# locuslab/icnn

Measured on AMD Instinct MI355X. Metric: inner-solves/sec (batch x iters), n=159 K=10, higher is better.
Workload: dtype f32 PICNN / f64 dual solve

## Files before the change

### icnn_amd/_lib.py

```python
import ctypes as C
import os

import torch

HERE = os.path.dirname(os.path.abspath(__file__))
LIB_PATH = os.path.join(HERE, "csrc", "libicnn_be.so")
if os.environ.get("ICNN_BE_LIB"):
    LIB_PATH = os.path.abspath(os.environ["ICNN_BE_LIB"])

ABI_VERSION = 12
MAX_LAYERS = 8
MAX_SLOTS = 31
MAX_ITERS = 64
MAX_ROUNDS = 128
VARIANT = {"dual": 0, "rl": 1, "pdipm": 2}
CUT_F32, CUT_F64 = 0, 1
ST_SINGULAR, ST_NONFINITE, ST_OVERFLOW, ST_UNFINISHED = 1, 2, 4, 8
ST_ERROR_MASK = ST_SINGULAR | ST_NONFINITE | ST_UNFINISHED | ST_OVERFLOW
FLAG_NO_CYCLE_SHORTCUT = 1
FLAG_TIME_SLICE = 2
FLAG_LOCKSTEP = 4
FLAG_TWO_KERNELS = 8
FLAG_PERSISTENT = 16
FLAG_F64_ENERGY = 32
# ... 8 lines not shown
DUAL_KERNELS = ["small", "body", "wide"]
ERRORS = {-1: "ICNN_BE_EINVAL (bad argument)", -2: "ICNN_BE_ELIMIT (size beyond a compiled-in limit)",
          -3: "ICNN_BE_ELAUNCH (HIP launch failed)"}

EXPORTS = [
    "icnn_be_abi_version", "icnn_be_last_hip_error", "icnn_be_struct_size", "icnn_be_dual_lds_bytes", "icnn_be_bundle_capacity", "icnn_be_scratch_bytes",
    "icnn_be_state_init",
    "icnn_be_dual_step", "icnn_be_fc_pack_floats", "icnn_be_fc_pack", "icnn_be_fc_fg",
    "icnn_be_solve_fc", "icnn_be_solve_fc_reset", "icnn_be_conv_pack_floats", "icnn_be_conv_work_floats", "icnn_be_conv_pack", "icnn_be_conv_fg", "icnn_be_solve_conv",
    "icnn_be_implicit_feed", "icnn_be_export_active", "icnn_be_adam_workspace_bytes", "icnn_be_adam_fc", "icnn_be_adam_fc_obs",
    "icnn_be_adam_fc_each", "icnn_be_debug_adam_each_plan",
    "icnn_be_fc_context_work_floats", "icnn_be_fc_context", "icnn_be_fc_context_stage", "icnn_be_fc_context_norm", "icnn_be_fc_clamp",
    "icnn_be_conv_context_work_floats", "icnn_be_conv_context", "icnn_be_conv_clamp",
    "icnn_be_debug_profile", "icnn_be_debug_profile_fc", "icnn_be_debug_profile_conv", "icnn_be_debug_profile_phases",
    "icnn_be_debug_fast_math", "icnn_be_debug_trace", "icnn_be_debug_solve_plan", "icnn_be_debug_adam_plan", "icnn_be_debug_dual_plan",
    "icnn_be_debug_shape_instance",
    "icnn_be_fc_grad_floats", "icnn_be_fc_surrogate_grad_work_floats", "icnn_be_fc_surrogate_grad",
    "icnn_be_conv_grad_floats", "icnn_be_conv_surrogate_grad_work_floats", "icnn_be_conv_surrogate_grad",
    "icnn_be_fc_context_bn_work_floats", "icnn_be_fc_context_bn", "icnn_be_conv_context_bn_work_floats", "icnn_be_conv_context_bn",
    "icnn_be_fc_surrogate_grad_bn", "icnn_be_conv_surrogate_grad_bn", "icnn_be_param_update",
    "icnn_be_gd_workspace_bytes", "icnn_be_fc_gd", "icnn_be_conv_gd",
    "icnn_be_rl_td", "icnn_be_rl_critic_update", "icnn_be_rl_bundle_solve",
    "icnn_be_ficnn_pack_floats", "icnn_be_ficnn_pack", "icnn_be_ficnn_context_work_floats", "icnn_be_ficnn_context",
    "icnn_be_ficnn_fg", "icnn_be_ficnn_gd", "icnn_be_solve_ficnn", "icnn_be_ficnn_grad_floats",
    "icnn_be_ficnn_surrogate_grad_work_floats", "icnn_be_ficnn_surrogate_grad",
    "icnn_be_feed_plan_work_bytes", "icnn_be_feed_plan", "icnn_be_feed_pad", "icnn_be_fc_surrogate_grad_dev",
    "icnn_be_conv_surrogate_grad_dev", "icnn_be_fc_context_bn_dev", "icnn_be_conv_context_bn_dev",
    "icnn_be_fc_surrogate_grad_dev_work_floats", "icnn_be_conv_surrogate_grad_dev_work_floats",
    "icnn_be_gd_feed_work_bytes", "icnn_be_gd_feed", "icnn_be_gd_feed_px_work_bytes", "icnn_be_gd_feed_px",
    "icnn_be_step_gate", "icnn_be_param_update_gated", "icnn_be_gated_copy",
    "icnn_be_replay_enqueue", "icnn_be_replay_sample",
# ... 283 lines not shown
    lib.icnn_be_implicit_feed.argtypes = [C.POINTER(State), C.c_void_p, C.c_int] + [C.c_void_p] * 6
    lib.icnn_be_implicit_feed.restype = C.c_int
    lib.icnn_be_export_active.argtypes = [C.POINTER(State)] + [C.c_void_p] * 6
    lib.icnn_be_export_active.restype = C.c_int
    lib.icnn_be_debug_fast_math.argtypes = [C.c_int, C.c_void_p, C.c_void_p, C.c_int, C.c_void_p]
    lib.icnn_be_debug_fast_math.restype = C.c_int
    lib.icnn_be_debug_solve_plan.argtypes = [C.POINTER(FcModel), C.POINTER(State), C.c_int, C.POINTER(C.c_int * 3)]
    lib.icnn_be_debug_solve_plan.restype = C.c_int
    lib.icnn_be_debug_profile_phases.restype = C.c_int
    lib.icnn_be_debug_adam_plan.argtypes = [C.POINTER(FcModel), C.POINTER(FcCtx), C.c_int, C.POINTER(C.c_int * 4)]
    lib.icnn_be_debug_adam_plan.restype = C.c_int
    lib.icnn_be_debug_dual_plan.argtypes = [C.POINTER(State), C.c_int, C.POINTER(C.c_int * 8)]
    lib.icnn_be_debug_dual_plan.restype = C.c_int
    lib.icnn_be_debug_shape_instance.argtypes = [C.POINTER(FcModel), C.POINTER(State)]
    lib.icnn_be_debug_shape_instance.restype = C.c_int
    lib.icnn_be_adam_workspace_bytes.argtypes = [C.c_int, C.c_int]
    lib.icnn_be_adam_workspace_bytes.restype = C.c_size_t
    lib.icnn_be_adam_fc.argtypes = [C.POINTER(FcModel), C.c_void_p, C.c_int, C.c_int] + [C.c_void_p] * 5
    lib.icnn_be_adam_fc.restype = C.c_int
    lib.icnn_be_adam_fc_each.argtypes = [C.POINTER(FcModel), C.c_void_p, C.c_int, C.c_int] + [C.c_void_p] * 5
    lib.icnn_be_adam_fc_each.restype = C.c_int
    lib.icnn_be_debug_adam_each_plan.argtypes = [C.POINTER(FcModel), C.c_int, C.POINTER(C.c_int * 2)]
    lib.icnn_be_debug_adam_each_plan.restype = C.c_int
    lib.icnn_be_adam_fc_obs.argtypes = [C.POINTER(FcModel), C.POINTER(FcCtx), C.c_void_p, C.c_int, C.c_int] + [C.c_void_p] * 5
    lib.icnn_be_adam_fc_obs.restype = C.c_int
    lib.icnn_be_fc_context_work_floats.argtypes = [C.POINTER(FcCtx), C.c_int]
    lib.icnn_be_fc_context_work_floats.restype = C.c_size_t
    lib.icnn_be_fc_context.argtypes = [C.POINTER(FcCtx), C.c_void_p, C.c_int, C.c_void_p, C.c_int, C.c_void_p, C.c_void_p]
    lib.icnn_be_fc_context.restype = C.c_int
    lib.icnn_be_fc_context_stage.argtypes = [C.POINTER(FcCtx), C.c_int, C.c_void_p, C.c_int, C.c_void_p, C.c_int, C.c_void_p,
# ... 260 lines not shown
def solve_plan(model, state, cus=0):
    out = (C.c_int * 3)()
    rc = load().icnn_be_debug_solve_plan(C.byref(model), C.byref(state), cus, C.byref(out))
    if rc < 0:
        check(rc, "icnn_be_debug_solve_plan")
    return (PATHS[rc],) + tuple(out)


def shape_instance(model, state):
    rc = load().icnn_be_debug_shape_instance(C.byref(model), C.byref(state))
    if rc < 0:
        check(rc, "icnn_be_debug_shape_instance")
    return SHAPE_INSTANCES[rc]


def adam_plan(model, batch, ctx=None):
    out = (C.c_int * 4)()
    rc = load().icnn_be_debug_adam_plan(C.byref(model), C.byref(ctx) if ctx is not None else None, int(batch), C.byref(out))
    if rc < 0:
        check(rc, "icnn_be_debug_adam_plan")
    return (ADAM_KERNELS[rc], out[0], out[1], bool(out[2]), bool(out[3]))


def adam_each_plan(model, batch):
    out = (C.c_int * 2)()
    rc = load().icnn_be_debug_adam_each_plan(C.byref(model), int(batch), C.byref(out))
    if rc < 0:
        check(rc, "icnn_be_debug_adam_each_plan")
    return (ADAM_KERNELS[rc], out[0], out[1])

# ... 9 lines not shown
```

### icnn_amd/csrc/be_api.hip

```cpp
#include <hip/hip_runtime.h>
#include <cmath>
#include <cstdlib>

#include <map>
#include <mutex>
#include <utility>

#include "be_api_check.h"
#include "be_kernels.h"
#include "icnn_be.h"

namespace {
thread_local hipError_t g_last = hipSuccess;

int fail(hipError_t e) {
    g_last = e;
    return e == hipErrorInvalidValue ? ICNN_BE_EINVAL : ICNN_BE_ELAUNCH;
}

int done(hipError_t e) { return e == hipSuccess ? 0 : fail(e); }
}

int icnn_be::api_done(hipError_t e) { return done(e); }

// ... 322 lines not shown
                                                    static_cast<hipStream_t>(stream), false,
                                                    icnn_be::SolveReset{1, nullptr, y0_fill}, &value);
    return e == hipSuccess ? p.rounds : fail(e);
}

int icnn_be_debug_solve_plan(const icnn_be_fc_model *model, const icnn_be_state *st, int cus, int out[3]) {
    if (!out) return ICNN_BE_EINVAL;
    if (int rc = check_fc_solve(model, st)) return rc;
    if (st->batch == 0) return ICNN_BE_EINVAL;
    const SolvePlan p = plan_fc_solve(*model, *st, cus > 0 ? cus : icnn_be::device_cus(), env_tile_budget());
    if (p.path < 0) return p.path;
    out[0] = p.per_wg; out[1] = p.budget; out[2] = p.rounds;
    return p.path;
}

int icnn_be_debug_shape_instance(const icnn_be_fc_model *model, const icnn_be_state *st) {
    if (model && st && st->cut_dtype == ICNN_BE_CUT_F64 && check_shape(st) == 0 && st->n == model->n && st->batch > 0 &&
        icnn_be::fc_check_model(*model) == 0)
        return ICNN_BE_SHAPE_GENERIC;
    if (int rc = check_fc_solve(model, st)) return rc;
    if (st->batch == 0) return ICNN_BE_EINVAL;
    const SolvePlan p = plan_fc_solve(*model, *st, icnn_be::device_cus(), env_tile_budget());
    if (p.path < 0) return p.path;
    if (p.path != ICNN_BE_PATH_TILE) return ICNN_BE_SHAPE_GENERIC;
    return icnn_be::fused_shape_instance(*model, *st, p.per_wg, p.budget);
}

size_t icnn_be_fc_context_work_floats(const icnn_be_fc_ctx *c, int batch) {
    if (!c || batch < 0 || icnn_be::ctx_check(*c) != 0) return 0;
    return icnn_be::ctx_work_floats(*c, batch);
// ... 505 lines not shown
```

### icnn_amd/csrc/be_fused.hip

```cpp
#include "be_dual_dev.h"
#include "be_dual_small_dev.h"
#include "be_picnn_fc_dev.h"
#include "be_picnn_fc_rows_dev.h"

namespace icnn_be {

namespace {

static_assert(NWAVE == TM, "one wave per sample in the dual phase");

struct FusedArgs {
    DualArgs da;
    FcArgs fa;
    int rounds, crow_off, samples_off, sample_bytes;
    int grouped;
    int group_cap, need_off;
    long long *trace;
    SolveReset reset;
};
typedef const __attribute__((address_space(4))) FusedArgs KArgs;

__device__ __forceinline__ void reset_sample(const icnn_be_state &st, const SolveReset &rs, int u, int lane) {
    const int n = st.n;
    double *yr = st.y + (size_t)u * n;
// ... 350 lines not shown
        !make_dual_args(args.da, st, nullptr, nullptr, 0, budget, st.slots, nullptr))
        return ICNN_BE_SHAPE_GENERIC;
    return pick_shape_instance(args, lay);
}

hipError_t launch_fused_fc_solve(const icnn_be_fc_model &m, const float *ctx, const icnn_be_state &st, float *f_work,
                                 float *g_work, long long *dual_prof, hipStream_t stream, int tile_rows, int budget,
                                 const SolveReset &reset) {
    if (budget > 0 && reset.on) return hipErrorInvalidValue;
    FusedTileLayout lay;
    if (!fused_tile_layout(m, st, tile_rows, budget, lay)) return hipErrorInvalidValue;
    FusedArgs args{};
    int fg_bytes = 0;
    if (fill_args(m, args.fa, fg_bytes) != 0) return hipErrorInvalidValue;
    args.fa.ctx = ctx; args.fa.y = st.y; args.fa.f = f_work; args.fa.g = g_work; args.fa.finished = st.skip_fg;
    args.fa.batch = st.batch; args.fa.prof = nullptr; args.fa.tile_rows = tile_rows;
    if (!make_dual_args(args.da, st, f_work, g_work, 0, budget, st.slots, dual_prof)) return hipErrorInvalidValue;
    args.rounds = st.iters > 0 ? st.iters : st.slots;
    args.crow_off = lay.crow_off; args.samples_off = 0; args.sample_bytes = lay.sample_bytes;
    args.grouped = lay.grouped; args.group_cap = lay.group_cap; args.need_off = lay.need_off;
    args.trace = dual_trace_buffer();
    args.reset = reset;
    const bool rl = st.variant == ICNN_BE_VARIANT_RL, big = st.slots > 15;
    auto kern = big ? (rl ? fused_fc_solve_kernel<true, 32> : fused_fc_solve_kernel<false, 32>)
                    : (rl ? fused_fc_solve_kernel<true, 16> : fused_fc_solve_kernel<false, 16>);
    if (st.variant == ICNN_BE_VARIANT_PDIPM) kern = big ? fused_fc_solve_kernel<false, 32, true> : fused_fc_solve_kernel<false, 16, true>;
    if (budget > 0) kern = big ? fused_fc_solve_kernel<false, 32, false, true> : fused_fc_solve_kernel<false, 16, false, true>;
    switch (pick_shape_instance(args, lay)) {
    case ICNN_BE_SHAPE_BIBTEX_KT16: kern = fused_fc_solve_kernel<false, 16, false, false, BibtexShape, 0>; break;
    case ICNN_BE_SHAPE_BIBTEX_KT32_GROUPED: kern = fused_fc_solve_kernel<false, 32, false, false, BibtexShape, 1>; break;
    default: break;
// ... 6 lines not shown
```

### icnn_amd/csrc/be_kernels.h

```cpp
#pragma once
#include <hip/hip_runtime.h>

#include "be_common.h"
#include "icnn_be.h"

namespace icnn_be {

struct DualArgs {
    icnn_be_state st;
    const void *f;
    const void *g;
    int round;
    int budget;
    int n_pad;
    int ldA;
    int rows;
    long long *prof;
    PairwisePlan plan;
};
constexpr int DUAL_PROF_PHASES = 16;
void set_dual_profile_buffer(long long *buf);
void set_fc_profile_buffer(long long *buf);
void set_conv_profile_buffer(long long *buf);

// ... 71 lines not shown
bool dual_step_small_fits(const icnn_be_state &st, int budget);
hipError_t launch_dual_step_small(const icnn_be_state &st, int round, const void *f, const void *g, hipStream_t stream);
struct DualStepPlan {
    int cut, kt, waves, variant, staged, kernel, lds, rows;
};
bool plan_dual_step(const icnn_be_state &st, int round, DualStepPlan &p);
void plan_dual_step_small(const icnn_be_state &st, DualStepPlan &p);

hipError_t launch_fast_math(int which, const double *x, double *out, int count, hipStream_t stream);
hipError_t launch_export_active(const icnn_be_state &st, const int *row_offset, void *G_rows, double *ys_rows, double *h_rows,
                                double *lam_rows, hipStream_t stream);
hipError_t launch_implicit_feed(const icnn_be_state &st, const double *y_true, int loss, const int *row_offset,
                                double *fd_y, double *fd_v, double *fd_c, int *fd_sample, hipStream_t stream);

int fc_check_model(const icnn_be_fc_model &m);
size_t fc_pack_floats(const icnn_be_fc_model &m);
int fc_pack(const icnn_be_fc_model &m, const float *const *w_yu, const float *const *w_zu, float *out);
hipError_t launch_fc_fg(const icnn_be_fc_model &m, const float *ctx, const double *y, int batch,
                        float *f, float *g, const int *finished, hipStream_t stream);

int ctx_check(const icnn_be_fc_ctx &c);
int conv_ctx_check(const icnn_be_conv_ctx &c);
size_t ctx_work_floats(const icnn_be_fc_ctx &c, int batch);
int ctx_stage_cols(const icnn_be_fc_ctx &c, int i);
int ctx_stage_ld(const icnn_be_fc_ctx &c, int i);
float *fc_ctx_u(const icnn_be_fc_ctx &c, int batch, float *work, int i, int *ld);
void fc_bn_widths(const icnn_be_fc_ctx &c, int *n);
hipError_t launch_fc_context(const icnn_be_fc_ctx &c, const float *x, int batch, float *ctx, int ctx_width, float *work,
                             hipStream_t stream, const icnn_be_bn_moving *mv = nullptr, int mode = ICNN_BE_BN_BATCH,
                             int updates = 0, const int *updates_dev = nullptr);
// ... 159 lines not shown
```

### icnn_amd/csrc/be_picnn_fc.hip

```cpp
#include "be_picnn_fc_dev.h"
#include "be_picnn_fc_rows_dev.h"

namespace icnn_be {

namespace {

__global__ __launch_bounds__(NTHREADS) void fc_fg_kernel(FcArgs a) {
    extern __shared__ __attribute__((aligned(16))) float lds[];
    fc_fg_tile(a, blockIdx.x, lds);
}

struct FgRowsArgs {
    FcArgs fa;
    RowsLayout lay;
    int per_wg;
};
__global__ __launch_bounds__(RTHREADS) void fc_fg_rows_kernel(FgRowsArgs a) {
#pragma clang fp contract(off)
    extern __shared__ __attribute__((aligned(16))) float lds[];
    const FcArgs &fa = a.fa;
    const int tid = threadIdx.x, wave = tid >> 6, lane = tid & 63;
    const int n = fa.n, RF = a.lay.row_floats;
    const int s_base = blockIdx.x * a.per_wg;
    const int batch = fa.batch - s_base < a.per_wg ? fa.batch - s_base : a.per_wg;
// ... 80 lines not shown
            if (e != hipSuccess) return e;
        } else {
            hipError_t e = launch_clamp(w + o.zu_f[i], (size_t)pad16(m.width[i - 1]), mode, stream);
            if (e != hipSuccess) return e;
        }
    }
    return hipSuccess;
}

int fc_check_model(const icnn_be_fc_model &m) {
    FcArgs a{};
    int lds = 0;
    return fill_args(m, a, lds);
}

}
```

### icnn_amd/csrc/be_picnn_fc_dev.h

```cpp
#pragma once
#include <hip/hip_runtime.h>

#include "be_common.h"
#include "be_kernels.h"
#include "icnn_be.h"

namespace icnn_be {

namespace {

constexpr int TM = 16;
constexpr int NWAVE = 16;
constexpr int NTHREADS = NWAVE * 64;

__host__ __device__ constexpr int pad16(int v) { return (v + 15) & ~15; }

struct FcArgs {
    int n, L;
    int width[ICNN_BE_MAX_LAYERS];
    float alpha;
    int action_box;
    int ctx_width;
    int yu_off[ICNN_BE_MAX_LAYERS], zu_off[ICNN_BE_MAX_LAYERS], gate_off[ICNN_BE_MAX_LAYERS];
    long long w_yu_f[ICNN_BE_MAX_LAYERS], w_yu_b[ICNN_BE_MAX_LAYERS];
    long long w_zu_f[ICNN_BE_MAX_LAYERS], w_zu_b[ICNN_BE_MAX_LAYERS];
    int zb_off[ICNN_BE_MAX_LAYERS], zb_ld[ICNN_BE_MAX_LAYERS];
    int ldY, ybuf_off, aop_off[ICNN_BE_MAX_LAYERS], gbuf_off, dl_off, lds_floats;
    const float *wpack, *ctx;
    const double *y;
    float *f, *g;
    const int *finished;
    int batch;
    int tile_rows;
    long long *prof;
};
constexpr int FC_PROF_PHASES = 16;

constexpr int PF = 5;
constexpr int TILE_RD = 2;
constexpr bool TILE_PAIR = false;
constexpr int TILE_STEP = (TILE_PAIR ? 2 : 1) * NWAVE;
__host__ __device__ constexpr int kblocks(int K) { return (pad16(K) / 16 + PF - 1) / PF * PF; }
// ... 48 lines not shown
    }
    o.total = at;
    return o;
}
inline PackOffsets pack_offsets(const icnn_be_fc_model &m) { return pack_offsets(m.n, m.n_layers, m.width); }

struct FcGeom {
    int n, L;
    int width[ICNN_BE_MAX_LAYERS];
    int ctx_width;
    int yu_off[ICNN_BE_MAX_LAYERS], zu_off[ICNN_BE_MAX_LAYERS], gate_off[ICNN_BE_MAX_LAYERS];
    long long w_yu_f[ICNN_BE_MAX_LAYERS], w_yu_b[ICNN_BE_MAX_LAYERS];
    long long w_zu_f[ICNN_BE_MAX_LAYERS], w_zu_b[ICNN_BE_MAX_LAYERS];
    int zb_off[ICNN_BE_MAX_LAYERS], zb_ld[ICNN_BE_MAX_LAYERS];
    int ldY, ybuf_off, aop_off[ICNN_BE_MAX_LAYERS], gbuf_off, dl_off, lds_floats;
};
constexpr int fc_geom(int n, int n_layers, const int *width, FcGeom &a) {
    const int L = n_layers - 1;
    if (L < 1 || n_layers > ICNN_BE_MAX_LAYERS || width[L] != 1 || n < 1) return ICNN_BE_EINVAL;
    a.n = n;
    a.L = L;
    int o = 0, lo = 0;
    for (int i = 0; i <= L; ++i) {
        if (width[i] < 1) return ICNN_BE_EINVAL;
        a.width[i] = width[i];
        a.yu_off[i] = o; o += n;
        a.zu_off[i] = o; o += width[i];
        a.gate_off[i] = -1;
        if (i > 0) { a.gate_off[i] = o; o += width[i - 1]; }
    }
    a.ctx_width = o;
    const PackOffsets po = pack_offsets(n, n_layers, width);
    for (int i = 0; i <= L; ++i) {
        a.w_yu_f[i] = po.yu_f[i]; a.w_yu_b[i] = po.yu_b[i];
        a.w_zu_f[i] = po.zu_f[i]; a.w_zu_b[i] = po.zu_b[i];
    }
    a.ldY = lds_pitch(n);
    a.ybuf_off = lo; lo += TM * a.ldY;
    for (int i = 0; i < L; ++i) { a.aop_off[i] = lo; lo += TM * a.ldY; }
    a.gbuf_off = lo; lo += TM * a.ldY;
    for (int i = 0; i < L; ++i) {
        a.zb_ld[i] = lds_pitch(width[i]);
        a.zb_off[i] = lo; lo += TM * a.zb_ld[i];
    }
    a.dl_off = lo; lo += TM * a.zb_ld[L - 1];
    a.lds_floats = lo;
    return 0;
}
template <typename Dst>
constexpr void fc_geom_copy(Dst &d, const FcGeom &g) {
    d.n = g.n; d.L = g.L; d.ctx_width = g.ctx_width;
    d.ldY = g.ldY; d.ybuf_off = g.ybuf_off; d.gbuf_off = g.gbuf_off; d.dl_off = g.dl_off; d.lds_floats = g.lds_floats;
    for (int i = 0; i < ICNN_BE_MAX_LAYERS; ++i) {
        d.width[i] = g.width[i];
        d.yu_off[i] = g.yu_off[i]; d.zu_off[i] = g.zu_off[i]; d.gate_off[i] = g.gate_off[i];
        d.w_yu_f[i] = g.w_yu_f[i]; d.w_yu_b[i] = g.w_yu_b[i]; d.w_zu_f[i] = g.w_zu_f[i]; d.w_zu_b[i] = g.w_zu_b[i];
        d.zb_off[i] = g.zb_off[i]; d.zb_ld[i] = g.zb_ld[i]; d.aop_off[i] = g.aop_off[i];
    }
}
template <typename A>
constexpr bool fc_geom_same(const A &a, const FcGeom &g) {
    bool ok = a.n == g.n && a.L == g.L && a.ctx_width == g.ctx_width && a.ldY == g.ldY && a.ybuf_off == g.ybuf_off &&
              a.gbuf_off == g.gbuf_off && a.dl_off == g.dl_off && a.lds_floats == g.lds_floats;
    for (int i = 0; i < ICNN_BE_MAX_LAYERS; ++i)
        ok = ok && a.width[i] == g.width[i] && a.yu_off[i] == g.yu_off[i] && a.zu_off[i] == g.zu_off[i] &&
             a.gate_off[i] == g.gate_off[i] && a.w_yu_f[i] == g.w_yu_f[i] && a.w_yu_b[i] == g.w_yu_b[i] &&
             a.w_zu_f[i] == g.w_zu_f[i] && a.w_zu_b[i] == g.w_zu_b[i] && a.zb_off[i] == g.zb_off[i] &&
// ... 107 lines not shown

template <typename Shape = DynShape, typename ArgsT>
__device__ __forceinline__ void fc_fg_tile(const ArgsT &a, int tile, float *lds) {
#pragma clang fp contract(off)
    const int tid = thread_id(), lane = tid & 63, wave = tid >> 6;
    const int r16 = lane & 15, q = lane >> 4;
    const auto &ge = Shape::fc(a);
    const int TR = a.tile_rows;
    const int s0 = tile * TR;
    const int rows = min(TR, a.batch - s0);
    const int n = ge.n, L = ge.L, C = ge.ctx_width, ldY = ge.ldY;
    const int npad = pad16(n);
    float *ybuf = lds + ge.ybuf_off;
    long long tick = ICNN_BE_PROF_ON(a.prof) ? (long long)__builtin_readcyclecounter() : 0;
    auto lap = [&](int phase) {
        if (ICNN_BE_PROF_ON(a.prof)) {
            const long long now = (long long)__builtin_readcyclecounter();
            if (lane == 0)
                atomicAdd(reinterpret_cast<unsigned long long *>(a.prof) +
                              ((size_t)tile * NWAVE + wave) * FC_PROF_PHASES + phase,
                          (unsigned long long)(now - tick));
            tick = now;
        }
    };

    int live = 1;
    if (a.finished) {
        live = 0;
        if (tid < rows) live = a.finished[s0 + tid] == 0;
    }
    const float *ctx = a.ctx + (size_t)s0 * C;
// ... 31 lines not shown
                const int j = j0 + 64 * k + lane;
                if (j < npad) {
                    const float v = a.action_box ? (float)(2.0 * yd[k] - 1.0) : (float)yd[k];
                    const bool ok = row_ok && j < n;
                    ybuf[r * ldY + j] = ok ? v : 0.f;
#pragma unroll
                    for (int i = 0; i < ICNN_BE_MAX_LAYERS; ++i)
                        if (i < L) lds[ge.aop_off[i] + r * ldY + j] = ok ? v * cu[k][i] : 0.f;
                }
            }
        }
    }
    __syncthreads();
    lap(0);

    const float *wyL = a.wpack + ge.w_yu_f[L];
    const float *wzL = a.wpack + ge.w_zu_f[L];
#pragma unroll(Shape::LAYER_UNROLL)
    for (int i = 0; i < L; ++i) {
        const int wi = ge.width[i], wpad = pad16(wi);
        const bool last = i == L - 1;
        float *zout = lds + ge.zb_off[i];
        const int ldo = ge.zb_ld[i];
        const int NT = wpad / 16, KBy = kblocks_tile(n);
        const float *Wy = a.wpack + ge.w_yu_f[i];
        for (int nt = wave; nt < NT; nt += TILE_STEP) {
            const int nt1 = TILE_PAIR && nt + NWAVE < NT ? nt + NWAVE : -1;
            f4 acc[2] = {{0.f, 0.f, 0.f, 0.f}, {0.f, 0.f, 0.f, 0.f}};
            float czu[2][4], cgt[2][4], wz[2];
            auto operands = [&] {
#pragma unroll
                for (int h = 0; h < (TILE_PAIR ? 2 : 1); ++h) {
                    const int tile = h == 0 ? nt : nt1;
                    const int col = tile * 16 + r16;
                    const int cc = tile >= 0 && col < wi ? col : 0;
                    wz[h] = wzL[last ? cc : 0];
#pragma unroll
                    for (int r = 0; r < 4; ++r) {
                        const int row = 4 * q + r;
                        const float *c = ctx + (size_t)(row < rows ? row : 0) * C;
                        czu[h][r] = c[ge.zu_off[i] + cc];
                        cgt[h][r] = c[ge.gate_off[i + 1] + cc];
// ... 17 lines not shown
                        const float z = act_fn(acc[h][r] + czu[h][r], a.alpha);
                        v = z * cgt[h][r];
                        const float gw = cgt[h][r] * wz[h];
                        d = gw * (v > 0.f ? 1.f : a.alpha);
                    }
                    zout[row * ldo + col] = v;
                    if (last) dl[row * ldo + col] = d;
                }
            }
        }
        lap(2 + 3 * i);
        __syncthreads();
        lap(3 + 3 * i);
    }

#pragma unroll(Shape::LAYER_UNROLL)
    for (int i = L - 1; i >= 0; --i) {
        const int wi = ge.width[i];
        const bool first = i == L - 1;
        const float *delta = first ? dl : lds + ge.zb_off[i];
        const int ldd = ge.zb_ld[i], KB = kblocks_tile(wi);
        const int NTy = npad / 16;
        {
            const float *Wt = a.wpack + ge.w_yu_b[i];
            const int wy = i > 0 ? NWAVE - 1 - wave : wave;
            for (int nt = wy; nt < NTy; nt += TILE_STEP) {
                const int nt1 = TILE_PAIR && nt + NWAVE < NTy ? nt + NWAVE : -1;
                f4 acc[2] = {{0.f, 0.f, 0.f, 0.f}, {0.f, 0.f, 0.f, 0.f}};
                float cyu[2][4], cyL[2][4], wy[2];
                const int offL = first ? ge.yu_off[L] : ge.yu_off[i];
                auto operands = [&] {
#pragma unroll
                    for (int h = 0; h < (TILE_PAIR ? 2 : 1); ++h) {
                        const int tile = h == 0 ? nt : nt1;
                        const int col = tile * 16 + r16;
                        const int cc = tile >= 0 && col < n ? col : 0;
                        wy[h] = wyL[first ? cc : 0];
#pragma unroll
                        for (int r = 0; r < 4; ++r) {
                            const int row = 4 * q + r;
                            const float *c = ctx + (size_t)(row < rows ? row : 0) * C;
                            cyu[h][r] = c[ge.yu_off[i] + cc];
                            cyL[h][r] = c[offL + cc];
                        }
                    }
                };
                gemm_tiles(delta, ldd, Wt, KB, NTy, nt, nt1, acc[0], acc[1], operands);
#pragma unroll
                for (int h = 0; h < 2; ++h) {
                    const int tile = h == 0 ? nt : nt1;
                    if (tile < 0) continue;
                    const int col = tile * 16 + r16;
#pragma unroll
                    for (int r = 0; r < 4; ++r) {
                        const int row = 4 * q + r;
                        if (row < rows && col < n) {
                            const float g_in = first ? cyL[h][r] * wy[h] : gbuf[row * ldY + col];
                            gbuf[row * ldY + col] = __builtin_fmaf(cyu[h][r], acc[h][r], g_in);
                        }
                    }
                }
            }
        }
        lap(i == 0 ? 11 : 8);
        if (i > 0) {
            const int wp = ge.width[i - 1];
            float *zprev = lds + ge.zb_off[i - 1];
            const int ldp = ge.zb_ld[i - 1];
            const float *Wt = a.wpack + ge.w_zu_b[i];
            const int NTp = pad16(wp) / 16;
            for (int nt = wave; nt < NTp; nt += TILE_STEP) {
                const int nt1 = TILE_PAIR && nt + NWAVE < NTp ? nt + NWAVE : -1;
                f4 acc[2] = {{0.f, 0.f, 0.f, 0.f}, {0.f, 0.f, 0.f, 0.f}};
                float cga[2][4];
                auto operands = [&] {
#pragma unroll
                    for (int h = 0; h < (TILE_PAIR ? 2 : 1); ++h) {
                        const int tile = h == 0 ? nt : nt1;
                        const int col = tile * 16 + r16;
                        const int cc = tile >= 0 && col < wp ? col : 0;
#pragma unroll
                        for (int r = 0; r < 4; ++r) {
                            const int row = 4 * q + r;
                            cga[h][r] = ctx[(size_t)(row < rows ? row : 0) * C + ge.gate_off[i] + cc];
                        }
                    }
                };
                gemm_tiles(delta, ldd, Wt, KB, NTp, nt, nt1, acc[0], acc[1], operands);
#pragma unroll
                for (int h = 0; h < 2; ++h) {
                    const int tile = h == 0 ? nt : nt1;
                    if (tile < 0) continue;
                    const int col = tile * 16 + r16;
#pragma unroll
                    for (int r = 0; r < 4; ++r) {
                        const int row = 4 * q + r;
                        float d = 0.f;
                        if (row < rows && col < wp) {
                            const float gate = cga[h][r];
                            const float ga = gate * acc[h][r];
                            d = ga * (zprev[row * ldp + col] > 0.f ? 1.f : a.alpha);
                        }
                        zprev[row * ldp + col] = d;
                    }
                }
            }
            lap(9);
        } else {
            const float *zl = lds + ge.zb_off[L - 1];
            const int ldz = ge.zb_ld[L - 1], wl = ge.width[L - 1];
            const int busy = NTy < NWAVE ? NTy : NWAVE, idle = NWAVE - busy;
            const int r0 = idle > 0 ? wave - busy : wave, rstep = idle > 0 ? idle : NWAVE;
            if (r0 >= 0)
                for (int r = r0; r < rows; r += rstep) {
                    const float *c = ctx + (size_t)r * C;
                    float part = 0.f;
                    for (int j = lane; j < wl; j += 64) part = __builtin_fmaf(zl[r * ldz + j], wzL[j], part);
                    for (int j = lane; j < n; j += 64) {
                        const float yy = ybuf[r * ldY + j] * c[ge.yu_off[L] + j];
                        part = __builtin_fmaf(yy, wyL[j], part);
                    }
                    const float e = wave_sum_f(part) + c[ge.zu_off[L]];
                    if (lane == 0) a.f[s0 + r] = e;
                }
            lap(7);
        }
        __syncthreads();
        lap(i == 0 ? 12 : 10);
    }

    const float gscale = a.action_box ? 2.f : 1.f;
    if (wave < rows)
        for (int j = lane; j < n; j += 64) a.g[(size_t)(s0 + wave) * n + j] = gscale * gbuf[wave * ldY + j];
    lap(13);
}


inline int fill_args(const icnn_be_fc_model &m, FcArgs &a, int &lds_bytes) {
    FcGeom g{};
    if (int rc = fc_geom(m.n, m.n_layers, m.width, g)) return rc;
    if (g.ctx_width != m.ctx_width) return ICNN_BE_EINVAL;
    fc_geom_copy(a, g);
    a.alpha = m.alpha;
    a.action_box = m.action_box;
    a.tile_rows = TM;
    lds_bytes = g.lds_floats * 4;
    if (lds_bytes > LDS_BYTES) return ICNN_BE_ELIMIT;
    a.wpack = m.wpack;
// ... 6 lines not shown
```

### include/icnn_be.h

```cpp
#ifndef ICNN_BE_H
#define ICNN_BE_H

#include <stddef.h>

#ifdef __cplusplus
extern "C" {
#endif

#if defined(__GNUC__)
#define ICNN_BE_API __attribute__((visibility("default")))
#else
#define ICNN_BE_API
#endif

#define ICNN_BE_ABI_VERSION 12
#define ICNN_BE_MAX_LAYERS 8
#define ICNN_BE_MAX_SLOTS 31
#define ICNN_BE_MAX_ITERS 64
#define ICNN_BE_MAX_ROUNDS 128

#define ICNN_BE_VARIANT_DUAL 0
#define ICNN_BE_VARIANT_RL 1
#define ICNN_BE_VARIANT_PDIPM 2

// ... 477 lines not shown

ICNN_BE_API void icnn_be_debug_profile(long long *device_buf);
ICNN_BE_API void icnn_be_debug_trace(long long *device_buf);
ICNN_BE_API int icnn_be_debug_profile_phases(void);
ICNN_BE_API int icnn_be_debug_fast_math(int which, const double *x, double *out, int count, void *stream);
ICNN_BE_API void icnn_be_debug_profile_fc(long long *device_buf);
ICNN_BE_API void icnn_be_debug_profile_conv(long long *device_buf);
ICNN_BE_API int icnn_be_debug_solve_plan(const icnn_be_fc_model *model, const icnn_be_state *st, int cus, int out[3]);
ICNN_BE_API int icnn_be_debug_adam_plan(const icnn_be_fc_model *model, const icnn_be_fc_ctx *cx, int batch, int out[4]);
ICNN_BE_API int icnn_be_debug_adam_each_plan(const icnn_be_fc_model *model, int batch, int out[2]);
ICNN_BE_API int icnn_be_debug_dual_plan(const icnn_be_state *st, int t, int out[8]);
#define ICNN_BE_SHAPE_GENERIC 0
#define ICNN_BE_SHAPE_BIBTEX_KT16 1
#define ICNN_BE_SHAPE_BIBTEX_KT32_GROUPED 2
ICNN_BE_API int icnn_be_debug_shape_instance(const icnn_be_fc_model *model, const icnn_be_state *st);


#define ICNN_BE_DDPG_MAX_OBS 600
#define ICNN_BE_DDPG_MAX_ACT 32
#define ICNN_BE_DDPG_MAX_HIDDEN 600
#define ICNN_BE_DDPG_STEP_INTS 4
#define ICNN_BE_DDPG_W_A2 0
#define ICNN_BE_DDPG_W_Y 1
#define ICNN_BE_DDPG_W_Q 2
#define ICNN_BE_DDPG_W_TD 3
#define ICNN_BE_DDPG_W_A 4
#define ICNN_BE_DDPG_W_QPI 5
#define ICNN_BE_DDPG_W_XA 6
#define ICNN_BE_DDPG_W_H2Q 7
#define ICNN_BE_DDPG_W_D3Q 8
// ... 238 lines not shown
```

Measured before the change: 45.20 million.

## Load-balance PICNN backward dE/dy tiles and energy rows across waves

Adds a compile-time work deal that assigns backward dE/dy tiles and energy-row dot products to the least-loaded wave, moving each layer's dE/dy work past the barrier so it overlaps the next delta GEMM. The last dE/dy_0 tile is kept in registers and fused into the final gradient store, and the energy computation handles two rows per pass with vectorized loads. This aims to remove wave imbalance and a separate gbuf read-back pass, at the cost of more register pressure and a more complex schedule. It also turns the fused path's profile buffer on and adds a debug export that reports the deal.

```diff
diff --git a/icnn_amd/_lib.py b/icnn_amd/_lib.py
--- a/icnn_amd/_lib.py
+++ b/icnn_amd/_lib.py
@@ -46,7 +46,7 @@
     "icnn_be_conv_context_work_floats", "icnn_be_conv_context", "icnn_be_conv_clamp",
     "icnn_be_debug_profile", "icnn_be_debug_profile_fc", "icnn_be_debug_profile_conv", "icnn_be_debug_profile_phases",
     "icnn_be_debug_fast_math", "icnn_be_debug_trace", "icnn_be_debug_solve_plan", "icnn_be_debug_adam_plan", "icnn_be_debug_dual_plan",
-    "icnn_be_debug_shape_instance",
+    "icnn_be_debug_shape_instance", "icnn_be_debug_fc_deal",
     "icnn_be_fc_grad_floats", "icnn_be_fc_surrogate_grad_work_floats", "icnn_be_fc_surrogate_grad",
     "icnn_be_conv_grad_floats", "icnn_be_conv_surrogate_grad_work_floats", "icnn_be_conv_surrogate_grad",
     "icnn_be_fc_context_bn_work_floats", "icnn_be_fc_context_bn", "icnn_be_conv_context_bn_work_floats", "icnn_be_conv_context_bn",
@@ -360,6 +360,8 @@
     lib.icnn_be_debug_dual_plan.restype = C.c_int
     lib.icnn_be_debug_shape_instance.argtypes = [C.POINTER(FcModel), C.POINTER(State)]
     lib.icnn_be_debug_shape_instance.restype = C.c_int
+    lib.icnn_be_debug_fc_deal.argtypes = [C.POINTER(FcModel), C.POINTER(C.c_int), C.c_int]
+    lib.icnn_be_debug_fc_deal.restype = C.c_int
     lib.icnn_be_adam_workspace_bytes.argtypes = [C.c_int, C.c_int]
     lib.icnn_be_adam_workspace_bytes.restype = C.c_size_t
     lib.icnn_be_adam_fc.argtypes = [C.POINTER(FcModel), C.c_void_p, C.c_int, C.c_int] + [C.c_void_p] * 5
@@ -650,6 +652,19 @@
     return SHAPE_INSTANCES[rc]
 
 
+UNIT_KINDS = ["fwd_y", "fwd_z", "delta", "dedy", "e"]
+
+
+def fc_deal(model):
+    lib = load()
+    count = lib.icnn_be_debug_fc_deal(C.byref(model), None, 0)
+    if count < 0:
+        check(count, "icnn_be_debug_fc_deal")
+    out = (C.c_int * (6 * count))()
+    lib.icnn_be_debug_fc_deal(C.byref(model), out, count)
+    return [(UNIT_KINDS[out[6 * k]],) + tuple(out[6 * k + 1:6 * k + 6]) for k in range(count)]
+
+
 def adam_plan(model, batch, ctx=None):
     out = (C.c_int * 4)()
     rc = load().icnn_be_debug_adam_plan(C.byref(model), C.byref(ctx) if ctx is not None else None, int(batch), C.byref(out))
diff --git a/icnn_amd/csrc/be_api.hip b/icnn_amd/csrc/be_api.hip
--- a/icnn_amd/csrc/be_api.hip
+++ b/icnn_amd/csrc/be_api.hip
@@ -360,6 +360,11 @@
     return p.path;
 }
 
+int icnn_be_debug_fc_deal(const icnn_be_fc_model *model, int *out, int cap) {
+    if (!model || cap < 0 || (cap > 0 && !out)) return ICNN_BE_EINVAL;
+    return icnn_be::fc_deal_units(*model, out, cap);
+}
+
 int icnn_be_debug_shape_instance(const icnn_be_fc_model *model, const icnn_be_state *st) {
     if (model && st && st->cut_dtype == ICNN_BE_CUT_F64 && check_shape(st) == 0 && st->n == model->n && st->batch > 0 &&
         icnn_be::fc_check_model(*model) == 0)
diff --git a/icnn_amd/csrc/be_fused.hip b/icnn_amd/csrc/be_fused.hip
--- a/icnn_amd/csrc/be_fused.hip
+++ b/icnn_amd/csrc/be_fused.hip
@@ -388,7 +388,7 @@
     int fg_bytes = 0;
     if (fill_args(m, args.fa, fg_bytes) != 0) return hipErrorInvalidValue;
     args.fa.ctx = ctx; args.fa.y = st.y; args.fa.f = f_work; args.fa.g = g_work; args.fa.finished = st.skip_fg;
-    args.fa.batch = st.batch; args.fa.prof = nullptr; args.fa.tile_rows = tile_rows;
+    args.fa.batch = st.batch; args.fa.prof = fc_profile_buffer(); args.fa.tile_rows = tile_rows;
     if (!make_dual_args(args.da, st, f_work, g_work, 0, budget, st.slots, dual_prof)) return hipErrorInvalidValue;
     args.rounds = st.iters > 0 ? st.iters : st.slots;
     args.crow_off = lay.crow_off; args.samples_off = 0; args.sample_bytes = lay.sample_bytes;
diff --git a/icnn_amd/csrc/be_kernels.h b/icnn_amd/csrc/be_kernels.h
--- a/icnn_amd/csrc/be_kernels.h
+++ b/icnn_amd/csrc/be_kernels.h
@@ -109,6 +109,7 @@
                                 double *fd_y, double *fd_v, double *fd_c, int *fd_sample, hipStream_t stream);
 
 int fc_check_model(const icnn_be_fc_model &m);
+int fc_deal_units(const icnn_be_fc_model &m, int *out, int cap);
 size_t fc_pack_floats(const icnn_be_fc_model &m);
 int fc_pack(const icnn_be_fc_model &m, const float *const *w_yu, const float *const *w_zu, float *out);
 hipError_t launch_fc_fg(const icnn_be_fc_model &m, const float *ctx, const double *y, int batch,
diff --git a/icnn_amd/csrc/be_picnn_fc.hip b/icnn_amd/csrc/be_picnn_fc.hip
--- a/icnn_amd/csrc/be_picnn_fc.hip
+++ b/icnn_amd/csrc/be_picnn_fc.hip
@@ -118,4 +118,47 @@
     return fill_args(m, a, lds);
 }
 
+
+int fc_deal_units(const icnn_be_fc_model &m, int *out, int cap) {
+    FcGeom g{};
+    if (int rc = fc_geom(m.n, m.n_layers, m.width, g)) return rc;
+    static_assert(FC_UNIT_FWD_Y == ICNN_BE_UNIT_FWD_Y && FC_UNIT_FWD_Z == ICNN_BE_UNIT_FWD_Z && FC_UNIT_DELTA == ICNN_BE_UNIT_DELTA &&
+                  FC_UNIT_DEDY == ICNN_BE_UNIT_DEDY && FC_UNIT_E == ICNN_BE_UNIT_E, "include/icnn_be.h");
+    const FcDeal &d = g.deal;
+    const int L = g.L, NTy = pad16(g.n) / 16;
+    int count = 0;
+    auto put = [&](int kind, int layer, int tile, int interval, int wave, int result) {
+        if (count < cap) {
+            const int rec[6] = {kind, layer, tile, interval, wave, result};
+            for (int k = 0; k < 6; ++k) out[6 * count + k] = rec[k];
+        }
+        ++count;
+    };
+    auto bwd = [&](int layer) { return 2 * L - 1 - layer; };
+    for (int i = 0; i < L; ++i) {
+        const int NT = pad16(g.width[i]) / 16;
+        for (int t = 0; t < NT; ++t) {
+            const int wave = fc_home_wave(t);
+            put(FC_UNIT_FWD_Y, i, t, i, wave, i);
+            if (i > 0) put(FC_UNIT_FWD_Z, i, t, i, wave, i);
+        }
+    }
+    for (int i = L - 1; i >= 0; --i) {
+        if (i > 0)
+            for (int t = 0; t < pad16(g.width[i - 1]) / 16; ++t) put(FC_UNIT_DELTA, i, t, bwd(i), fc_home_wave(t), bwd(i));
+        for (int t = 0; t < NTy; ++t) {
+            if (!d.bwd_moved) {
+                put(FC_UNIT_DEDY, i, t, bwd(i), fc_home_wave_dedy(i, t), bwd(i));
+                continue;
+            }
+            for (int w = 0; w < NWAVE; ++w)
+                if (d.dy_mask[i][w] >> t & 1) put(FC_UNIT_DEDY, i, t, bwd(i > 0 ? i - 1 : 0), w, i > 0 ? bwd(i - 1) : 2 * L);
+        }
+    }
+    for (int r = 0; r < TM; ++r)
+        for (int w = 0; w < NWAVE; ++w)
+            if (d.e_mask[w] >> r & 1) put(FC_UNIT_E, L, r, bwd(0), w, bwd(0));
+    return count;
 }
+
+}
diff --git a/icnn_amd/csrc/be_picnn_fc_dev.h b/icnn_amd/csrc/be_picnn_fc_dev.h
--- a/icnn_amd/csrc/be_picnn_fc_dev.h
+++ b/icnn_amd/csrc/be_picnn_fc_dev.h
@@ -14,6 +14,12 @@
 constexpr int NTHREADS = NWAVE * 64;
 
 __host__ __device__ constexpr int pad16(int v) { return (v + 15) & ~15; }
+
+struct FcDeal {
+    int bwd_moved;
+    unsigned short dy_mask[ICNN_BE_MAX_LAYERS][NWAVE];
+    unsigned short e_mask[NWAVE];
+};
 
 struct FcArgs {
     int n, L;
@@ -26,6 +32,7 @@
     long long w_zu_f[ICNN_BE_MAX_LAYERS], w_zu_b[ICNN_BE_MAX_LAYERS];
     int zb_off[ICNN_BE_MAX_LAYERS], zb_ld[ICNN_BE_MAX_LAYERS];
     int ldY, ybuf_off, aop_off[ICNN_BE_MAX_LAYERS], gbuf_off, dl_off, lds_floats;
+    FcDeal deal;
     const float *wpack, *ctx;
     const double *y;
     float *f, *g;
@@ -104,7 +111,52 @@
     long long w_zu_f[ICNN_BE_MAX_LAYERS], w_zu_b[ICNN_BE_MAX_LAYERS];
     int zb_off[ICNN_BE_MAX_LAYERS], zb_ld[ICNN_BE_MAX_LAYERS];
     int ldY, ybuf_off, aop_off[ICNN_BE_MAX_LAYERS], gbuf_off, dl_off, lds_floats;
+    FcDeal deal;
 };
+
+enum { FC_UNIT_FWD_Y = 0, FC_UNIT_FWD_Z = 1, FC_UNIT_DELTA = 2, FC_UNIT_DEDY = 3, FC_UNIT_E = 4 };
+constexpr int FC_E_ROW_COST = 2;
+constexpr int fc_deal_pick(const int *load) {
+    int best = NWAVE - 1;
+    for (int w = NWAVE - 2; w >= 0; --w)
+        if (load[w] < load[best]) best = w;
+    return best;
+}
+constexpr FcDeal fc_deal(int n, int L, const int *width) {
+    FcDeal d{};
+    const int NTy = pad16(n) / 16;
+    d.bwd_moved = NTy <= NWAVE;
+    for (int i = L - 1; i >= 0; --i) {
+        int load[NWAVE] = {};
+        if (i > 0)
+            for (int t = 0; t < pad16(width[i - 1]) / 16; ++t) load[t % NWAVE] += kblocks_tile(width[i]);
+        if (d.bwd_moved) {
+            if (i == 0)
+                for (int t = 0; t < NTy; ++t) {
+                    d.dy_mask[0][t] = (unsigned short)(1u << t);
+                    load[t] += kblocks_tile(width[0]);
+                }
+            if (i + 1 < L)
+                for (int t = 0; t < NTy; ++t) {
+                    const int w = fc_deal_pick(load);
+                    d.dy_mask[i + 1][w] |= (unsigned short)(1u << t);
+                    load[w] += kblocks_tile(width[i + 1]);
+                }
+        } else {
+            for (int t = 0; t < NTy; ++t) load[i > 0 ? NWAVE - 1 - t % NWAVE : t % NWAVE] += kblocks_tile(width[i]);
+        }
+        if (i == 0)
+            for (int r = 0; r < TM; ++r) {
+                const int w = fc_deal_pick(load);
+                d.e_mask[w] |= (unsigned short)(1u << r);
+                load[w] += FC_E_ROW_COST;
+            }
+    }
+    return d;
+}
+__host__ __device__ constexpr int fc_home_wave(int t) { return t % NWAVE; }
+__host__ __device__ constexpr int fc_home_wave_dedy(int layer, int t) { return layer > 0 ? NWAVE - 1 - t % NWAVE : t % NWAVE; }
+
 constexpr int fc_geom(int n, int n_layers, const int *width, FcGeom &a) {
     const int L = n_layers - 1;
     if (L < 1 || n_layers > ICNN_BE_MAX_LAYERS || width[L] != 1 || n < 1) return ICNN_BE_EINVAL;
@@ -135,12 +187,14 @@
     }
     a.dl_off = lo; lo += TM * a.zb_ld[L - 1];
     a.lds_floats = lo;
+    a.deal = fc_deal(n, L, width);
     return 0;
 }
 template <typename Dst>
 constexpr void fc_geom_copy(Dst &d, const FcGeom &g) {
     d.n = g.n; d.L = g.L; d.ctx_width = g.ctx_width;
     d.ldY = g.ldY; d.ybuf_off = g.ybuf_off; d.gbuf_off = g.gbuf_off; d.dl_off = g.dl_off; d.lds_floats = g.lds_floats;
+    d.deal = g.deal;
     for (int i = 0; i < ICNN_BE_MAX_LAYERS; ++i) {
         d.width[i] = g.width[i];
         d.yu_off[i] = g.yu_off[i]; d.zu_off[i] = g.zu_off[i]; d.gate_off[i] = g.gate_off[i];
@@ -278,7 +332,7 @@
     float *ybuf = lds + ge.ybuf_off;
     long long tick = ICNN_BE_PROF_ON(a.prof) ? (long long)__builtin_readcyclecounter() : 0;
     auto lap = [&](int phase) {
-        if (ICNN_BE_PROF_ON(a.prof)) {
+        if (ICNN_BE_PROF_ON(a.prof) && phase < FC_PROF_PHASES) {
             const long long now = (long long)__builtin_readcyclecounter();
             if (lane == 0)
                 atomicAdd(reinterpret_cast<unsigned long long *>(a.prof) +
@@ -340,18 +394,22 @@
     __syncthreads();
     lap(0);
 
+    static_assert(!TILE_PAIR, "the dE/dy_0 unit carries ONE accumulator across the last barrier");
+    const auto &deal = ge.deal;
+    const int wv = __builtin_amdgcn_readfirstlane(wave);
     const float *wyL = a.wpack + ge.w_yu_f[L];
     const float *wzL = a.wpack + ge.w_zu_f[L];
+    const int KBy = kblocks_tile(n);
 #pragma unroll(Shape::LAYER_UNROLL)
     for (int i = 0; i < L; ++i) {
         const int wi = ge.width[i], wpad = pad16(wi);
         const bool last = i == L - 1;
         float *zout = lds + ge.zb_off[i];
         const int ldo = ge.zb_ld[i];
-        const int NT = wpad / 16, KBy = kblocks_tile(n);
+        const int NT = wpad / 16;
         const float *Wy = a.wpack + ge.w_yu_f[i];
-        for (int nt = wave; nt < NT; nt += TILE_STEP) {
-            const int nt1 = TILE_PAIR && nt + NWAVE < NT ? nt + NWAVE : -1;
+        for (int nt = fc_home_wave(wave); nt < NT; nt += TILE_STEP) {
+            const int nt1 = -1;
             f4 acc[2] = {{0.f, 0.f, 0.f, 0.f}, {0.f, 0.f, 0.f, 0.f}};
             float czu[2][4], cgt[2][4], wz[2];
             auto operands = [&] {
@@ -399,124 +457,169 @@
         lap(3 + 3 * i);
     }
 
+    const int NTy = npad / 16;
+    const bool bmoved = deal.bwd_moved;
+    f4 gacc = {0.f, 0.f, 0.f, 0.f};
+    float gcyu[4] = {0.f, 0.f, 0.f, 0.f};
+    int gtile = -1;
+    auto dy_unit = [&](int j, int nt, bool defer) {
+        const bool first = j == L - 1;
+        const float *delta = first ? dl : lds + ge.zb_off[j];
+        f4 acc = {0.f, 0.f, 0.f, 0.f}, none = {0.f, 0.f, 0.f, 0.f};
+        float cyu[4], cyL[4], wy;
+        const int offL = first ? ge.yu_off[L] : ge.yu_off[j];
+        const int col = nt * 16 + r16;
+        auto operands = [&] {
+            const int cc = col < n ? col : 0;
+            wy = wyL[first ? cc : 0];
+#pragma unroll
+            for (int r = 0; r < 4; ++r) {
+                const int row = 4 * q + r;
+                const float *c = ctx + (size_t)(row < rows ? row : 0) * C;
+                cyu[r] = c[ge.yu_off[j] + cc];
+                cyL[r] = c[offL + cc];
+            }
+        };
+        gemm_tiles(delta, ge.zb_ld[j], a.wpack + ge.w_yu_b[j], kblocks_tile(ge.width[j]), NTy, nt, -1, acc, none, operands);
+#pragma unroll
+        for (int r = 0; r < 4; ++r) {
+            const int row = 4 * q + r;
+            if (row < rows && col < n) {
+                const float g_in = first ? cyL[r] * wy : gbuf[row * ldY + col];
+                if (!defer) gbuf[row * ldY + col] = __builtin_fmaf(cyu[r], acc[r], g_in);
+                else if (first) gbuf[row * ldY + col] = g_in;
+            }
+            gcyu[r] = defer ? cyu[r] : gcyu[r];
+        }
+        if (defer) {
+            gacc = acc;
+            gtile = nt;
+        }
+    };
 #pragma unroll(Shape::LAYER_UNROLL)
     for (int i = L - 1; i >= 0; --i) {
         const int wi = ge.width[i];
         const bool first = i == L - 1;
         const float *delta = first ? dl : lds + ge.zb_off[i];
         const int ldd = ge.zb_ld[i], KB = kblocks_tile(wi);
-        const int NTy = npad / 16;
-        {
-            const float *Wt = a.wpack + ge.w_yu_b[i];
-            const int wy = i > 0 ? NWAVE - 1 - wave : wave;
-            for (int nt = wy; nt < NTy; nt += TILE_STEP) {
-                const int nt1 = TILE_PAIR && nt + NWAVE < NTy ? nt + NWAVE : -1;
-                f4 acc[2] = {{0.f, 0.f, 0.f, 0.f}, {0.f, 0.f, 0.f, 0.f}};
-                float cyu[2][4], cyL[2][4], wy[2];
-                const int offL = first ? ge.yu_off[L] : ge.yu_off[i];
-                auto operands = [&] {
-#pragma unroll
-                    for (int h = 0; h < (TILE_PAIR ? 2 : 1); ++h) {
-                        const int tile = h == 0 ? nt : nt1;
-                        const int col = tile * 16 + r16;
-                        const int cc = tile >= 0 && col < n ? col : 0;
-                        wy[h] = wyL[first ? cc : 0];
-#pragma unroll
-                        for (int r = 0; r < 4; ++r) {
-                            const int row = 4 * q + r;
-                            const float *c = ctx + (size_t)(row < rows ? row : 0) * C;
-                            cyu[h][r] = c[ge.yu_off[i] + cc];
-                            cyL[h][r] = c[offL + cc];
-                        }
-                    }
-                };
-                gemm_tiles(delta, ldd, Wt, KB, NTy, nt, nt1, acc[0], acc[1], operands);
-#pragma unroll
-                for (int h = 0; h < 2; ++h) {
-                    const int tile = h == 0 ? nt : nt1;
-                    if (tile < 0) continue;
-                    const int col = tile * 16 + r16;
-#pragma unroll
-                    for (int r = 0; r < 4; ++r) {
-                        const int row = 4 * q + r;
-                        if (row < rows && col < n) {
-                            const float g_in = first ? cyL[h][r] * wy[h] : gbuf[row * ldY + col];
-                            gbuf[row * ldY + col] = __builtin_fmaf(cyu[h][r], acc[h][r], g_in);
-                        }
-                    }
-                }
-            }
-        }
-        lap(i == 0 ? 11 : 8);
+        if (!bmoved)
+            for (int nt = fc_home_wave_dedy(i, wave); nt < NTy; nt += TILE_STEP) dy_unit(i, nt, false);
         if (i > 0) {
             const int wp = ge.width[i - 1];
             float *zprev = lds + ge.zb_off[i - 1];
             const int ldp = ge.zb_ld[i - 1];
             const float *Wt = a.wpack + ge.w_zu_b[i];
             const int NTp = pad16(wp) / 16;
-            for (int nt = wave; nt < NTp; nt += TILE_STEP) {
-                const int nt1 = TILE_PAIR && nt + NWAVE < NTp ? nt + NWAVE : -1;
-                f4 acc[2] = {{0.f, 0.f, 0.f, 0.f}, {0.f, 0.f, 0.f, 0.f}};
-                float cga[2][4];
+            for (int nt = fc_home_wave(wave); nt < NTp; nt += TILE_STEP) {
+                f4 acc = {0.f, 0.f, 0.f, 0.f}, none = {0.f, 0.f, 0.f, 0.f};
+                float cga[4];
+                const int col = nt * 16 + r16;
                 auto operands = [&] {
-#pragma unroll
-                    for (int h = 0; h < (TILE_PAIR ? 2 : 1); ++h) {
-                        const int tile = h == 0 ? nt : nt1;
-                        const int col = tile * 16 + r16;
-                        const int cc = tile >= 0 && col < wp ? col : 0;
-#pragma unroll
-                        for (int r = 0; r < 4; ++r) {
-                            const int row = 4 * q + r;
-                            cga[h][r] = ctx[(size_t)(row < rows ? row : 0) * C + ge.gate_off[i] + cc];
+                    const int cc = col < wp ? col : 0;
+#pragma unroll
+                    for (int r = 0; r < 4; ++r) {
+                        const int row = 4 * q + r;
+                        cga[r] = ctx[(size_t)(row < rows ? row : 0) * C + ge.gate_off[i] + cc];
+                    }
+                };
+                gemm_tiles(delta, ldd, Wt, KB, NTp, nt, -1, acc, none, operands);
+#pragma unroll
+                for (int r = 0; r < 4; ++r) {
+                    const int row = 4 * q + r;
+                    float d = 0.f;
+                    if (row < rows && col < wp) {
+                        const float gate = cga[r];
+                        const float ga = gate * acc[r];
+                        d = ga * (zprev[row * ldp + col] > 0.f ? 1.f : a.alpha);
+                    }
+                    zprev[row * ldp + col] = d;
+                }
+            }
+        }
+        if (bmoved && i == 0 && deal.dy_mask[0][wv]) dy_unit(0, __builtin_ctz(deal.dy_mask[0][wv]), true);
+        lap(i == 0 ? 10 : 8);
+        if (bmoved && i + 1 < L)
+            for (unsigned m = deal.dy_mask[i + 1][wv]; m; m &= m - 1) dy_unit(i + 1, __builtin_ctz(m), false);
+        if (i == 0) lap(11);
+        if (i == 0) {
+            const float *zl = lds + ge.zb_off[L - 1];
+            const int ldz = ge.zb_ld[L - 1], wl = ge.width[L - 1];
+            unsigned m = rows > 0 ? deal.e_mask[wv] & ((1u << rows) - 1u) : 0u;
+            while (m) {
+                int rr[2];
+                rr[0] = rr[1] = __builtin_ctz(m);
+                m &= m - 1;
+                const bool two = m != 0;
+                if (two) {
+                    rr[1] = __builtin_ctz(m);
+                    m &= m - 1;
+                }
+                const float *c[2] = {ctx + (size_t)rr[0] * C, ctx + (size_t)rr[1] * C};
+                float part[2] = {0.f, 0.f}, cy[2][4], wyv[4], czL[2];
+                auto y_loads = [&](int j0) {
+#pragma unroll
+                    for (int k = 0; k < 4; ++k) {
+                        const int j = j0 + 64 * k + lane, jc = j < n ? j : 0;
+                        wyv[k] = wyL[jc];
+#pragma unroll
+                        for (int h = 0; h < 2; ++h) cy[h][k] = c[h][ge.yu_off[L] + jc];
+                    }
+                };
+                y_loads(0);
+#pragma unroll
+                for (int h = 0; h < 2; ++h) czL[h] = c[h][ge.zu_off[L]];
+                for (int j0 = 0; j0 < wl; j0 += 256) {
+                    float wzv[4], zv[2][4];
+#pragma unroll
+                    for (int k = 0; k < 4; ++k) {
+                        const int j = j0 + 64 * k + lane, jc = j < wl ? j : 0;
+                        wzv[k] = wzL[jc];
+#pragma unroll
+                        for (int h = 0; h < 2; ++h) zv[h][k] = zl[rr[h] * ldz + jc];
+                    }
+#pragma unroll
+                    for (int k = 0; k < 4; ++k)
+#pragma unroll
+                        for (int h = 0; h < 2; ++h)
+                            part[h] = j0 + 64 * k + lane < wl ? __builtin_fmaf(zv[h][k], wzv[k], part[h]) : part[h];
+                }
+                for (int j0 = 0; j0 < n; j0 += 256) {
+                    if (j0 > 0) y_loads(j0);
+#pragma unroll
+                    for (int k = 0; k < 4; ++k) {
+                        const int j = j0 + 64 * k + lane, jc = j < n ? j : 0;
+#pragma unroll
+                        for (int h = 0; h < 2; ++h) {
+                            const float yy = ybuf[rr[h] * ldY + jc] * cy[h][k];
+                            part[h] = j < n ? __builtin_fmaf(yy, wyv[k], part[h]) : part[h];
                         }
                     }
-                };
-                gemm_tiles(delta, ldd, Wt, KB, NTp, nt, nt1, acc[0], acc[1], operands);
+                }
 #pragma unroll
                 for (int h = 0; h < 2; ++h) {
-                    const int tile = h == 0 ? nt : nt1;
-                    if (tile < 0) continue;
-                    const int col = tile * 16 + r16;
-#pragma unroll
-                    for (int r = 0; r < 4; ++r) {
-                        const int row = 4 * q + r;
-                        float d = 0.f;
-                        if (row < rows && col < wp) {
-                            const float gate = cga[h][r];
-                            const float ga = gate * acc[h][r];
-                            d = ga * (zprev[row * ldp + col] > 0.f ? 1.f : a.alpha);
-                        }
-                        zprev[row * ldp + col] = d;
-                    }
-                }
-            }
-            lap(9);
-        } else {
-            const float *zl = lds + ge.zb_off[L - 1];
-            const int ldz = ge.zb_ld[L - 1], wl = ge.width[L - 1];
-            const int busy = NTy < NWAVE ? NTy : NWAVE, idle = NWAVE - busy;
-            const int r0 = idle > 0 ? wave - busy : wave, rstep = idle > 0 ? idle : NWAVE;
-            if (r0 >= 0)
-                for (int r = r0; r < rows; r += rstep) {
-                    const float *c = ctx + (size_t)r * C;
-                    float part = 0.f;
-                    for (int j = lane; j < wl; j += 64) part = __builtin_fmaf(zl[r * ldz + j], wzL[j], part);
-                    for (int j = lane; j < n; j += 64) {
-                        const float yy = ybuf[r * ldY + j] * c[ge.yu_off[L] + j];
-                        part = __builtin_fmaf(yy, wyL[j], part);
-                    }
-                    const float e = wave_sum_f(part) + c[ge.zu_off[L]];
-                    if (lane == 0) a.f[s0 + r] = e;
-                }
+                    const float e = wave_sum_f(part[h]) + czL[h];
+                    if (lane == 0 && (h == 0 || two)) a.f[s0 + rr[h]] = e;
+                }
+            }
             lap(7);
         }
         __syncthreads();
-        lap(i == 0 ? 12 : 10);
+        lap(i == 0 ? 12 : 9);
     }
 
     const float gscale = a.action_box ? 2.f : 1.f;
-    if (wave < rows)
-        for (int j = lane; j < n; j += 64) a.g[(size_t)(s0 + wave) * n + j] = gscale * gbuf[wave * ldY + j];
+    if (!bmoved) {
+        if (wave < rows)
+            for (int j = lane; j < n; j += 64) a.g[(size_t)(s0 + wave) * n + j] = gscale * gbuf[wave * ldY + j];
+    } else if (gtile >= 0) {
+        const int col = gtile * 16 + r16;
+#pragma unroll
+        for (int r = 0; r < 4; ++r) {
+            const int row = 4 * q + r;
+            if (row < rows && col < n)
+                a.g[(size_t)(s0 + row) * n + col] = gscale * __builtin_fmaf(gcyu[r], gacc[r], gbuf[row * ldY + col]);
+        }
+    }
     lap(13);
 }
 
diff --git a/include/icnn_be.h b/include/icnn_be.h
--- a/include/icnn_be.h
+++ b/include/icnn_be.h
@@ -515,6 +515,12 @@
 #define ICNN_BE_SHAPE_BIBTEX_KT16 1
 #define ICNN_BE_SHAPE_BIBTEX_KT32_GROUPED 2
 ICNN_BE_API int icnn_be_debug_shape_instance(const icnn_be_fc_model *model, const icnn_be_state *st);
+#define ICNN_BE_UNIT_FWD_Y 0
+#define ICNN_BE_UNIT_FWD_Z 1
+#define ICNN_BE_UNIT_DELTA 2
+#define ICNN_BE_UNIT_DEDY 3
+#define ICNN_BE_UNIT_E 4
+ICNN_BE_API int icnn_be_debug_fc_deal(const icnn_be_fc_model *model, int *out, int cap);
 
 
 #define ICNN_BE_DDPG_MAX_OBS 600
```

After: 46.12 million, median of 6. 1.02x the previous value.
